# vmoens/mujoco-torch

Hardware: AMD Instinct MI355X
Metric: env-steps/sec (higher is better)
Workload: dtype f64

## Files before the change

### mujoco-torch_amd/csrc/mjh_device.h

```cpp
#pragma once
#include <hip/hip_runtime.h>
#include <stdint.h>

#include "../../include/mjhip.h"

#define MJH_WAVE 64
#define MJH_MAX_DEPTH 128
#define MJH_CHAIN_PRE 3

#define mjMINVAL 1e-15
#define mjMAXVAL 1e10
#define mjMINIMP 1e-4
#define mjMAXIMP 0.9999
#define MINVAL_CACHED ((float)1e-15)

enum { JNT_FREE = 0, JNT_BALL = 1, JNT_SLIDE = 2, JNT_HINGE = 3 };
enum { DSBL_CONSTRAINT = 1 << 0, DSBL_SPRING = 1 << 5, DSBL_DAMPER = 1 << 6, DSBL_GRAVITY = 1 << 7,
       DSBL_CLAMPCTRL = 1 << 8, DSBL_WARMSTART = 1 << 9, DSBL_ACTUATION = 1 << 11, DSBL_REFSAFE = 1 << 12,
       DSBL_EULERDAMP = 1 << 15 };
enum { INT_EULER = 0, INT_RK4 = 1, SOL_CG = 1, SOL_NEWTON = 2, CONE_ELLIPTIC = 1 };
enum { CAM_FIXED = 0, CAM_TRACK = 1, CAM_TRACKCOM = 2, CAM_TARGETBODY = 3, CAM_TARGETBODYCOM = 4 };
enum { GAIN_FIXED = 0, GAIN_AFFINE = 1, GAIN_MUSCLE = 2, BIAS_NONE = 0, BIAS_AFFINE = 1, BIAS_MUSCLE = 2 };
enum { DYN_NONE = 0, DYN_INTEGRATOR = 1, DYN_FILTER = 2, DYN_FILTEREXACT = 3, DYN_MUSCLE = 4 };
#define INLINE_CHOL_MAX 16
// ... 111 lines not shown
  const int* dof_act_id;
  const REAL* dof_act_coef;
  const int* dof_frc_lim;
  const REAL* dof_frc_range;
  const int* dof_act_rot;
  const int* act_ent_adr;
  const int* act_ent_dof;
  const REAL* act_ent_coef;
  const int* act_ent_rot;
  const REAL* ten_J0;
  const REAL* ten_JTAJ;
  int has_ten_armature;
  int con_direct;
  int con_general;
  int act_simple;
  int act_has_rot;
  float inv_nv;
  const int* dof_limrow;
  const int* lim_dof;
  int sol_qm_lds;
  int con_rows;
  int nt_all;
  int all_handoff;
  int lds_diet;
  int crow_by_con;
  int sol2_row_cap;
  int pair_cull_on;
  int sol2_incr;
  int sol2_hs;
  const REAL* crow_par;
  const int* crow_info;
  int ncrow;
  const int* con_body;
  const unsigned long long* con_dmask;
  const REAL* pair_cull;
  const int* cvx_pairs;
  int ncvxpair;
};

__device__ __forceinline__ int lane_id() { return (int)(threadIdx.x & (MJH_WAVE - 1)); }

__device__ __forceinline__ void wave_sync() {
  __builtin_amdgcn_fence(__ATOMIC_RELEASE, "workgroup", "local");
  __builtin_amdgcn_wave_barrier();
  __builtin_amdgcn_fence(__ATOMIC_ACQUIRE, "workgroup", "local");
}
// ... 316 lines not shown
```

### mujoco-torch_amd/csrc/mjh_kernels.h

```cpp
#pragma once
#include <cstring>
#include "mjh_device.h"

template <typename REAL>
struct LdsView {
  REAL* base;
  const LdsOff* off;
#define X(n, c, p) __device__ __forceinline__ REAL* n() const { return base + off->n; }
  MJH_LDS_ARRAYS(X, _)
#undef X
};

#ifndef MJH_NO_NT
#define MJH_NT_STORE(v, p) __builtin_nontemporal_store((v), (p))
#else
#define MJH_NT_STORE(v, p) (*(p) = (v))
#endif
template <typename MM>
inline int lds_carve(const MM& m, int phase_bit, LdsOff& o, int* kv_defer_ok = nullptr) {
  int off = 0;
#define X(n, c, p) o.n = off; if ((p) & phase_bit) off += (((c) + 1) & ~1);
  MJH_LDS_ARRAYS(X, m)
#undef X
  if (phase_bit == PH_CON) {
// ... 78 lines not shown
    o.act = off; off += ev(m.na);
    o.act_dot = off; off += ev(m.na);
    o.con_dist = off; off += ev(m.ncand);
    o.i_con_act = off; off += ev(m.ncon);
    o.i_crow_act = off; off += ev(m.ncon);
    const int rows0 = off, nj = ev(nd * m.nv), n3 = ev(3 * m.ngeom), n9 = ev(9 * m.ngeom);
    o.efc_J = o.efc_Jc = rows0;
    if (n3 + n9 > nj) return -1;
    o.geom_xpos = rows0; o.geom_xmat = rows0 + n3;
    off += nj;
    const int ov = off;
    int ca = ov;
    o.subtree_com = ca; ca += ev(3 * m.nbody);
    o.cdof = ca; ca += ev(6 * m.nv);
    o.con_pos = ca; ca += ev(3 * m.ncand);
    o.con_frame = ca; ca += ev(9 * m.ncand);
    int sa = ov;
    o.efc_D = sa; sa += ev(nd);
    o.efc_aref = sa; sa += ev(nd);
    o.r_vs = sa; sa += ev(m.nv);
    o.r_vs2 = sa; sa += ev(m.nv);
    o.r_pg = sa; sa += ev(2 * m.nv);
    o.r_fs = sa; sa += ev(nd + m.nl);
    const int qpos_at = sa;
    o.qpos = sa; sa += ev(m.nq);
    off = ca > sa ? ca : sa;
    int ta = rows0;
#define X(n, c, p) if ((p) & PH_SOL2T) { o.n = ta; ta += (((c) + 1) & ~1); }
    MJH_LDS_ARRAYS(X, m)
#undef X
    if (ta > qpos_at) return -1;
  }
  if (phase_bit == PH_CRB) {
    const int nn = ((m.nv * m.nv + 1) & ~1);
    if (m.nv <= 32) { o.qLD = 0; if (off < nn) off = nn; }
    else { o.qLD = off; off += nn; }
  }
  return off;
}

template <typename REAL>
struct DevData {
#define X(n) REAL* n;
  MJH_DATA_REALS(X)
#undef X
#define X(n) int32_t* n;
// ... 412 lines not shown
  } else {
#pragma unroll
    for (int k = 0; k < NMAX; k++) T.t[k] = (k < n && valid && k <= i) ? A[(i * (i + 1)) / 2 + k] : (REAL)0;
  }
#pragma unroll
  for (int j = 0; j < NMAX; j++) {
    if (j < n) {
      const REAL sj = dof_read<W, NMAX>(T.t[j], j);
      const REAL dj = r_sqrt<REAL>(sj > (REAL)1e-12 ? sj : (REAL)1e-12);
      const REAL lij = (i == j) ? dj : ((i > j && valid) ? T.t[j] / dj : (REAL)0);
      if (i >= j) T.t[j] = lij;
#pragma unroll
      for (int k = j + 1; k < NMAX; k++) {
        const REAL lkj = dof_read<W, NMAX>(lij, k);
        T.t[k] = (i == j) ? lkj : ((i > j) ? T.t[k] - lij * lkj : T.t[k]);
      }
    }
  }
  REAL dg = 1;
#pragma unroll
  for (int k = 0; k < NMAX; k++) dg = (k == i) ? T.t[k] : dg;
  T.inv = valid ? 1 / dg : (REAL)0;
}
template <int W, typename REAL, int NMAX>
__device__ __forceinline__ void chol_pack_big(TriPack<REAL, NMAX>& T, REAL* colbuf, int n) {
  static_assert(NMAX > 16 && NMAX <= 32 && NMAX <= W, "one lane per row");
  const int i = sub_lane<W>();
  const bool valid = i < n;
#pragma unroll
  for (int j = 0; j < NMAX; j++) {
    if (j < n) {
      const REAL sj = sub_read<W>(T.t[j], j) + (REAL)1e-10;
      const REAL dj = r_sqrt<REAL>(sj);
      const REAL lij = (i == j) ? dj : ((i > j && valid) ? T.t[j] / dj : (REAL)0);
      if (i >= j) T.t[j] = lij;
      REAL* col = colbuf + (j & 1) * NMAX;
      if (i < NMAX) col[i] = lij;
      constexpr int CH = 8;
#pragma unroll
      for (int k0 = 0; k0 < NMAX; k0 += CH) {
        if (k0 + CH - 1 > j) {
          REAL c[CH];
#pragma unroll
          for (int t = 0; t < CH; t++) c[t] = (k0 + t > j && k0 + t < NMAX) ? col[k0 + t] : (REAL)0;
#pragma unroll
          for (int t = 0; t < CH; t++) {
            if (k0 + t > j && k0 + t < NMAX) {
              T.t[k0 + t] = (i == j) ? c[t] : ((i > j) ? T.t[k0 + t] - lij * c[t] : T.t[k0 + t]);
              asm volatile("" : "+v"(T.t[k0 + t]));
            }
          }
        }
      }
    }
  }
  REAL dg = 1;
#pragma unroll
  for (int k = 0; k < NMAX; k++) dg = (k == i) ? T.t[k] : dg;
  T.inv = valid ? 1 / dg : (REAL)0;
}

template <int W, typename REAL, int NMAX>
__device__ __forceinline__ void chol_factor_solve_n(const REAL* A, const REAL* b, REAL* x, int n) {
  TriPack<REAL, NMAX> T;
  chol_factor_pack<W, REAL, NMAX>(A, T, n);
  const int i = sub_lane<W>();
  const REAL xi = tri_solve<W, REAL, NMAX>(T, i < n ? b[i] : (REAL)0, n);
  if (i < n) x[i] = xi;
  wave_sync();
}
template <int W, typename REAL, int NLO = 0, int NHI = 16>
__device__ __forceinline__ void chol_factor_solve(const REAL* A, const REAL* b, REAL* x, int n) {
  if (NLO <= 8 && (NHI <= 8 || n <= 8)) { if constexpr (NLO <= 8) chol_factor_solve_n<W, REAL, 8>(A, b, x, n); }
  else if (NLO <= 12 && NHI > 8 && (NHI <= 12 || n <= 12)) { if constexpr (NLO <= 12 && NHI > 8) chol_factor_solve_n<W, REAL, 12>(A, b, x, n); }
  else { if constexpr (NHI > 12) chol_factor_solve_n<W, REAL, 16>(A, b, x, n); }
}

template <int W, bool APACKED, typename REAL, int NMAX>
__device__ __forceinline__ void chol_factor_reg(const REAL* A, REAL* L, int n) {
  const int i = sub_lane<W>();
  REAL row[NMAX];
#pragma unroll
// ... 571 lines not shown
          for (int i = 0; i < 9; i++) xmb[i] = S.xmat()[9 * b + i];
        }
#pragma unroll
        for (int r = 0; r < 3; r++) {
          const REAL a[3] = {xmb[r], xmb[3 + r], xmb[6 + r]};
          REAL c[3];
          cross3(a, off, c);
          for (int k = 0; k < 3; k++) { S.cdof()[6 * (d + r) + k] = a[k]; S.cdof()[6 * (d + r) + 3 + k] = c[k]; }
        }
      } else if (t == JNT_HINGE) {
        REAL c[3];
        cross3(S.xaxis() + 3 * j, off, c);
        for (int k = 0; k < 3; k++) { S.cdof()[6 * d + k] = S.xaxis()[3 * j + k]; S.cdof()[6 * d + 3 + k] = c[k]; }
      } else {
        for (int k = 0; k < 3; k++) { S.cdof()[6 * d + k] = 0; S.cdof()[6 * d + 3 + k] = S.xaxis()[3 * j + k]; }
      }
    }
    wave_sync();
    STAMP(6);
    if (!(DEFER && W > 16 && M.kv_defer)) com_stores();
    STAMP(7);
  }

  template <bool FUSED = false, int MAXN = (W == 16 ? 16 : 32)>
  __device__ __forceinline__ void crb_factor() {
    const int l = lane_here();
    const int nb = M.nbody, nv = M.nv;
    STAMP0();
    if (!FUSED) {
      REAL* const dst[2] = {S.cinert(), S.cdof()};
      const REAL* const src[2] = {out.cinert, out.cdof};
      const int cnt[2] = {10 * nb, 6 * nv};
      multi_load<W, 2, 3>(dst, src, cnt, e);
    }
    wave_sync();
    STAMP(11);
    for (int w = l; w < nb * 10; w += W) {
      const int b = w / 10, k = w - 10 * b;
      REAL acc = 0;
      if (b > 0) {
        const int end = M.body_subtree_end[b];
        for (int d = end - 1; d >= b; d--) acc += S.cinert()[10 * d + k];
      }
      S.crb()[w] = acc;
    }
    wave_sync();
    STAMP(12);
// ... 8 lines not shown
#pragma unroll
      for (int k = 0; k < 6; k++) s += S.crb_cdof()[6 * i + k] * S.cdof()[6 * j + k];
      if (i == j) s = s + M.dof_armature[i];
      S.qMp()[tri_at<true>(i, j, nv)] = s;
    }
    wave_sync();
    if (M.has_ten_armature) {
      for (int w = l; w < (nv * (nv + 1)) / 2; w += W) S.qMp()[w] = S.qMp()[w] + M.ten_JTAJ[w];
      wave_sync();
    }
    if (out.qM) {
      REAL* gM = out.qM + e * nv * nv;
      for (int w = l; w < nv * nv; w += W) {
        int i, j;
        split_index(w, nv, M.inv_nv, i, j);
        const int hi = i > j ? i : j, lo = i > j ? j : i;
        gM[w] = S.qMp()[(hi * (hi + 1)) / 2 + lo];
      }
    }
    STAMP(14);
    putnt(out.crb, S.crb(), 10 * nb);
    wave_sync();
    STAMP(15);
    chol_factor<W, REAL, MAXN, true>(S.qMp(), S.qLD(), nv);
    STAMP(16);
    put(out.qLD, S.qLD(), nv * nv);
    STAMP(17);
  }

  __device__ __forceinline__ static void plane_sphere_(const REAL* n, const REAL* ppos, const REAL* spos, REAL r, REAL& dist, REAL* pos) {
    const REAL d[3] = {spos[0] - ppos[0], spos[1] - ppos[1], spos[2] - ppos[2]};
    dist = dot3(d, n) - r;
#pragma unroll
    for (int i = 0; i < 3; i++) pos[i] = spos[i] - n[i] * (r + (REAL)0.5 * dist);
  }
  __device__ __forceinline__ static void sphere_sphere_(const REAL* p1, REAL r1, const REAL* p2, REAL r2, REAL& dist, REAL* pos, REAL* n) {
#pragma unroll
    for (int i = 0; i < 3; i++) n[i] = p2[i] - p1[i];
    REAL d = normalize_n<REAL, 3>(n);
    if (d == 0) { n[0] = 1; n[1] = 0; n[2] = 0; }
    d = d - (r1 + r2);
#pragma unroll
    for (int i = 0; i < 3; i++) pos[i] = p1[i] + n[i] * (r1 + d * (REAL)0.5);
    dist = d;
  }
  __device__ __forceinline__ static void closest_segment_point(const REAL* a, const REAL* b, const REAL* pt, REAL* o) {
// ... 2035 lines not shown
    wave_sync();
    row_store<W>(fin.qpos, S.tmp_nq(), M.nq, e);
    row_store<W>(fin.qvel, S.tmp_nv(), M.nv, e);
    if (l == 0 && fin.time) fin.time[e] = time0 + dt;
  }

  template <bool DEFER = false, bool KEEPG = false, bool XK = KEEPG>
  __device__ __forceinline__ void run_kin() {
    STAMP0();
    load_qpos(true);
    wave_sync();
    STAMP(1);
    const bool com_first = XK && (__builtin_popcount((unsigned)blockIdx.x & (unsigned)KA.xswap_k) & 1) != 0;
    kinematics<DEFER, KEEPG, XK>(KA.rk_stage <= 0, com_first);
    if (!com_first) com_pos<DEFER>();
  }
  __device__ __forceinline__ void run_crb() { crb_factor<false>(); }
  __device__ __forceinline__ void run_con() {
    STAMP0();
    if (M.ncon > 0) collision<0, false, true>();
    if (KA.stages & 0x78) make_constraint();
    if (M.ncon > 0 && !(FRIC && M.topk) && !consts_done_) contact_const_stores();
  }
  template <int NMAX>
  __device__ __forceinline__ void sol2_prefetch(Sol2Pre<REAL, NMAX>& P) {
    const int l = lane_here();
    const int nq = M.nq, nv = M.nv, na = M.na;
    const bool dof = l < nv;
    P.f = (dof && out.qfrc_smooth) ? out.qfrc_smooth[e * nv + l] : (REAL)0;
    {
      const REAL* gL = out.qLD + e * nv * nv;
#pragma unroll
      for (int k = 0; k < NMAX; k++) P.T.t[k] = (dof && k < nv) ? (k <= l ? gL[l * nv + k] : gL[k * nv + l]) : (REAL)0;
    }
    P.T.inv = 0;
    const REAL* gq = KA.cur.qpos + e * nq;
#pragma unroll
    for (int j = 0; j < 2; j++) P.qp[j] = l + W * j < nq ? gq[l + W * j] : (REAL)0;
    P.ac = 0; P.ad = 0;
    if (l < na) { const REAL* ga = KA.state_from_cur ? KA.cur.act : in.act; P.ac = ga ? ga[e * na + l] : (REAL)0; P.ad = out.act_dot ? out.act_dot[e * na + l] : (REAL)0; }
    P.warm = (dof && KA.warm_src && M.nefc > 0) ? KA.warm_src[e * nv + l] : (REAL)0;
  }
  template <int NMAX>
  __device__ __forceinline__ void make_constraint_cs(Sol2Pre<REAL, NMAX>& pre, Sol2Con<REAL>& C) {
    const int l = lane_here();
#if MJH_CS_PF >= 2
    {
      const REAL* gq = KA.cur.qpos + e * M.nq;
#pragma unroll
      for (int j = 0; j < 2; j++) pre.qp[j] = l + W * j < M.nq ? gq[l + W * j] : (REAL)0;
    }
#endif
    const int nv = M.nv, nefc = M.nefc, nl = M.nl, ncon = M.ncon, rows = M.con_rows;
    const bool elliptic = M.cone == CONE_ELLIPTIC;
    if (!KA.state_from_cur && KA.do_step) for (int i = l; i < nv; i += W) S.qvel()[i] = checked(S.qvel()[i], (REAL)0);
    REAL lpos = 0, linvw = 0;
    int lj = 0;
    C.jl = 0; C.ldof = 0;
    if (l < nl) {
      lj = M.lim_jnt[l];
      C.ldof = M.jnt_dofadr[lj];
    }
    {
      const int qa = l < nl ? M.jnt_qposadr[lj] : 0;
      const int srcl = (int)(lane_id() & ~(W - 1)) + (qa & (W - 1));
      const REAL q0 = __shfl(pre.qp[0], srcl, MJH_WAVE), q1 = __shfl(pre.qp[1], srcl, MJH_WAVE);
// ... 42 lines not shown
      jac_dof_root(cpos, root1, on1, d, jp1, jr1);
      const REAL dp[3] = {jp2[0] - jp1[0], jp2[1] - jp1[1], jp2[2] - jp1[2]};
      const REAL dr[3] = {jr2[0] - jr1[0], jr2[1] - jr1[1], jr2[2] - jr1[2]};
      REAL diff[6];
#pragma unroll
      for (int r = 0; r < 3; r++) {
        diff[r] = fr[3 * r] * dp[0] + fr[3 * r + 1] * dp[1] + fr[3 * r + 2] * dp[2];
        diff[3 + r] = fr[3 * r] * dr[0] + fr[3 * r + 1] * dr[1] + fr[3 * r + 2] * dr[2];
      }
      REAL* const dst = Jc + (a * rows) * nv + d;
      if (dim == 1) {
        dst[0] = diff[0];
      } else if (!elliptic) {
        const int nedge = 2 * (dim - 1);
        for (int ed = 0; ed < nedge; ed++) {
          const REAL f = fric[ed >> 1] * ((ed & 1) ? (REAL)-1 : (REAL)1);
          dst[ed * nv] = diff[0] + diff[1 + (ed >> 1)] * f;
        }
      } else {
        for (int r = 0; r < dim; r++) dst[r * nv] = diff[r];
      }
    }
#if MJH_CS_PF == 2
    sol2_prefetch<NMAX>(pre);
#endif
    wave_sync();
    STAMP(25);
    C.Dl = 0; C.arl = 0;
    for (int r = l; r < nefc; r += W) {
      REAL solref[2], solimp[5];
      REAL pos = 0, pos_norm = 0, invweight = 0, jv = 0;
      int crow = -1;
      if (r < nl) {
        pos = lpos; pos_norm = lpos; invweight = linvw;
        solref[0] = M.jnt_solref[2 * lj]; solref[1] = M.jnt_solref[2 * lj + 1];
#pragma unroll
        for (int i = 0; i < 5; i++) solimp[i] = M.jnt_solimp[5 * lj + i];
        jv = 0 + C.jl * S.qvel()[C.ldof];
      } else {
        const int q = r - nl, ncr = M.ncrow;
        const int info = M.crow_info[q];
        const REAL* P = M.crow_par + q;
        solref[0] = P[0]; solref[1] = P[ncr];
#pragma unroll
        for (int i = 0; i < 5; i++) solimp[i] = P[(2 + i) * ncr];
        invweight = P[7 * ncr];
        const int c = info & 0xffff, sub = (info >> 16) & 0xff;
// ... 34 lines not shown
      const REAL* Jc = S.efc_Jc();
      REAL* gC = gJ + nl * nv;
      for (int c = 0; c < M.ncon; c++) {
        const int at = slot[c];
        for (int sub = 0; sub < rows; sub += 4) {
          REAL v[4];
#pragma unroll
          for (int t = 0; t < 4; t++) v[t] = (at >= 0 && sub + t < rows && dof) ? Jc[(at * rows + sub + t) * nv + l] : (REAL)0;
#pragma unroll
          for (int t = 0; t < 4; t++) if (sub + t < rows && dof) MJH_NT_STORE(v[t], &gC[(c * rows + sub + t) * nv + l]);
        }
      }
    }
    if (out.efc_frictionloss) for (int r = l; r < nefc; r += W) MJH_NT_STORE((REAL)0, &out.efc_frictionloss[e * nefc + r]);
    if (M.ncon > 0) contact_const_stores();
  }
  template <int NMAX, int RPL, bool ONE = false, bool HANDOFF = false>
  __device__ __forceinline__ void run_con_sol2() {
    static_assert(W == 32 && !FRIC && !DIRECT, "plain constraint stage, two environments per wavefront");
    Sol2Pre<REAL, NMAX> pre;
    Sol2Con<REAL> con;
    STAMP0();
    collision<NMAX, HANDOFF>(&pre);
#if MJH_CS_PF == 1
    sol2_prefetch<NMAX>(pre);
#endif
    make_constraint_cs<NMAX>(pre, con);
#if MJH_CS_PF == 3
    if (HANDOFF && ho_on_) {
      __builtin_amdgcn_fence(__ATOMIC_RELEASE, "workgroup");
      __builtin_amdgcn_fence(__ATOMIC_ACQUIRE, "workgroup");
    }
    sol2_prefetch<NMAX>(pre);
#endif
    wave_sync();
    run_sol2<NMAX, RPL, false, true, ONE>(&pre, &con);
  }
  template <bool FLUID, bool FUSED = false, bool DEFER = false>
  __device__ __forceinline__ void run_vel() {
    STAMP0();
    velocity<FLUID, FUSED, DEFER>();
    if (KA.stages & 0x60) actuation<FLUID>();
    velocity_stores<DEFER>();
  }

  __device__ __forceinline__ void run_sol() {
    const int l = lane_here();
    const int nq = M.nq, nv = M.nv, na = M.na;
    STAMP0();
    load_factor_and_accelerate((KA.stages & 0x40) != 0);
    if (!(KA.stages & 0x40)) return;
    STAMP(53);
    if (M.nefc == 0) {
      for (int d = l; d < nv; d += W) S.qacc()[d] = S.qacc_smooth()[d];
      wave_sync();
      put(out.qacc, S.qacc(), nv);
    } else {
      solve();
    }
    integrate_tail();
  }

  template <int NMAX>
  __device__ __forceinline__ void load_damping_rows(TriPack<REAL, NMAX>& Hh) {
    const int l = lane_here();
    const int nv = M.nv;
    const REAL* gM = out.qM + e * nv * nv;
#pragma unroll
    for (int k = 0; k < NMAX; k++) Hh.t[k] = (l < nv && k <= l) ? gM[k * nv + l] : (REAL)0;
  }
  template <int NLO = 0, int NHI = (1 << 30)>
  __device__ __forceinline__ void integrate_tail() {
    const int l = lane_here();
    const int nq = M.nq, nv = M.nv, na = M.na;
    if (!KA.do_step) return;
    rebind();
    const REAL dt = M.timestep;
    const REAL time0 = in.time ? in.time[e] : (REAL)0;
    const int rk = KA.rk_stage;
    if (rk < 0) {
      const REAL* qacc = S.qacc();
      constexpr bool REGSOL = NHI <= 32;
      if (!(M.disableflags & DSBL_EULERDAMP)) {
        if constexpr (REGSOL && NLO > 16) {
          TriPack<REAL, NHI> Hh;
          load_damping_rows<NHI>(Hh);
          const REAL dd = l < nv ? M.timestep * M.dof_damping[l] : (REAL)0;
          const REAL rhs = l < nv ? S.qfrc_smooth()[l] + (M.nefc ? S.qfrc_constraint()[l] : (in.qfrc_constraint ? in.qfrc_constraint[e * nv + l] : (REAL)0)) : (REAL)0;
#pragma unroll
          for (int k = 0; k < NHI; k++) Hh.t[k] = (k == l) ? Hh.t[k] + dd : Hh.t[k];
          chol_pack_big<W, REAL, NHI>(Hh, S.chol_col(), nv);
          const REAL x = tri_solve<W, REAL, NHI>(Hh, rhs, nv);
          if (l < nv) S.s_Mgrad()[l] = x;
          wave_sync();
        } else {
        REAL* const Hp = REGSOL ? S.H2() : S.H();
        for (int w = l; w < (nv * (nv + 1)) / 2; w += W) {
          int i, j;
          tri_unpack(w, i, j);
          const REAL mw = out.qM[e * nv * nv + i * nv + j];
          Hp[w] = (i == j) ? mw + M.timestep * M.dof_damping[i] : mw;
        }
        for (int d = l; d < nv; d += W) S.s_grad()[d] = S.qfrc_smooth()[d] + (M.nefc ? S.qfrc_constraint()[d] : (in.qfrc_constraint ? in.qfrc_constraint[e * nv + d] : (REAL)0));
        wave_sync();
        if (NLO <= 16 && (NHI <= 16 || nv <= 16)) {
          if constexpr (NLO <= 16) chol_factor_solve<W, REAL, NLO, (NHI < 16 ? NHI : 16)>(Hp, S.s_grad(), S.s_Mgrad(), nv);
        } else {
          if constexpr (NHI > 16 && !REGSOL) {
            chol_factor<W, REAL, 16, true>(S.H(), S.HL(), nv);
            chol_inv_diag<W, false>(S.HL(), S.HL_inv(), nv);
            wave_sync();
            chol_solve<W, false>(S.HL(), S.HL_inv(), S.s_grad(), S.s_Mgrad(), nv);
          }
        }
        }
// ... 26 lines not shown
      for (int i = l; i < nv; i += W) S.tmp_nv2()[i] = a * S.qvel()[i];
      wave_sync();
      for (int i = l; i < nq; i += W) S.qpos()[i] = S.tmp_nq()[i];
      wave_sync();
      integrate_pos(S.qpos(), S.tmp_nv2(), dt, S.tmp_nq());
      for (int i = l; i < na; i += W) KA.nxt.act[e * na + i] = S.act()[i] + (a * S.act_dot()[i]) * dt;
      for (int i = l; i < nv; i += W) KA.nxt.qvel[e * nv + i] = S.s_pgrad()[i] + (a * S.qacc()[i]) * dt;
      wave_sync();
      row_store<W>(KA.nxt.qpos, S.tmp_nq(), nq, e);
      return;
    }
    for (int i = l; i < nv; i += W) { S.s_mv()[i] = RW.sum_qacc[e * nv + i]; S.tmp_nv2()[i] = RW.sum_qvel[e * nv + i]; }
    for (int i = l; i < na; i += W) S.act_dot()[i] = RW.sum_actdot[e * na + i];
    for (int i = l; i < nq; i += W) S.qpos()[i] = S.tmp_nq()[i];
    wave_sync();
    advance(S.qpos(), S.s_pgrad(), S.act(), time0, S.act_dot(), S.s_mv(), S.tmp_nv2());
  }

  template <int NMAX>
  __device__ __forceinline__ REAL tri_solve2(const TriPack<REAL, NMAX>& T, REAL bi) const {
    return tri_solve<W, REAL, NMAX>(T, bi, M.nv);
  }

  template <int NMAX, int RPL, bool NEWTON_ONLY = false, bool CS = false, bool ONE = false>
  __device__ __forceinline__ void run_sol2(const Sol2Pre<REAL, NMAX>* pre = nullptr, const Sol2Con<REAL>* con = nullptr) {
    static_assert(W == 32 || W == 16, "two or four environments per wavefront");
    static_assert(!CS || (W == 32 && !NEWTON_ONLY), "the fused constraint + solver kernel runs two environments per wavefront");
    constexpr bool NEWT = NMAX <= 16;
    const int l = lane_here();
    const int nq = M.nq, nv = M.nv, na = M.na, nefc = M.nefc, nl = M.nl, nd = nefc - nl;
    const bool dof = l < nv, lim = l < nl;
    const bool solving = (KA.stages & 0x40) != 0;
    const bool from_in = !KA.state_from_cur;
    const bool newton = NEWTON_ONLY ? NEWT : (NEWT && M.solver == SOL_NEWTON);
    STAMP0();
    if (KA.row_lo >= 0 && !KA.scan_marks) {
      int rows_active = 0;
      if (solving && nefc > 0) {
        const int ncon = M.ncon;
        const bool elliptic = M.cone == CONE_ELLIPTIC;
        for (int base = 0; base < ncon; base += W) {
          const int c = base + l;
          int rows = 0;
          if (c < ncon) {
            const int dim = M.con_dim[c];
            const bool act = (out.contact_dist[e * ncon + c] - (M.topk ? out.contact_includemargin[e * ncon + c] : M.con_includemargin[c])) < 0;
            rows = act ? (dim == 1 ? 1 : (elliptic ? dim : 2 * (dim - 1))) : 0;
// ... 155 lines not shown
            if (r < nda) { Dd[j] = S.efc_D()[r]; ard[j] = S.efc_aref()[r]; }
          }
          STAMP(83);
        } else if (hsp) {
          STAMP(83);
          const REAL* hJ = hsp + 1 + M.ncon + 2 * nd;
          REAL* dJ = S.efc_Jc();
          const int n = nda * nv;
          for (int i0 = 0; i0 < n; i0 += 16 * W) {
            REAL v[16];
#pragma unroll
            for (int t = 0; t < 16; t++) { const int i = i0 + t * W + l; v[t] = i < n ? hJ[i] : (REAL)0; }
#pragma unroll
            for (int t = 0; t < 16; t++) { const int i = i0 + t * W + l; if (i < n) dJ[i] = v[t]; }
          }
        } else {
#pragma unroll
        for (int j = 0; j < RPL; j++) {
          const int r = l + W * j;
          if (r < nda) { const int x = rsrc[r]; Dd[j] = out.efc_D[e * nefc + x]; ard[j] = out.efc_aref[e * nefc + x]; }
        }
        STAMP(83);
        gather_rows<16>(S.efc_Jc(), gJ, rsrc, nda * nv);
        }
      }
    }
    STAMP(70);
    {
      REAL dg = 1;
#pragma unroll
      for (int k = 0; k < NMAX; k++) dg = (k == l) ? T.t[k] : dg;
      T.inv = dof ? 1 / dg : (REAL)0;
    }
    const REAL qs = tri_solve2<NMAX>(T, f);
    if (dof && out.qacc_smooth) out.qacc_smooth[e * nv + l] = qs;
    STAMP(71);
    if (!solving) return;
    REAL qacc = qs, qfrc = 0;
    if (nefc > 0) {
      const REAL* gM = out.qM + e * nv * nv;
      const REAL scale = (REAL)(M.meaninertia * (double)(nv > 1 ? nv : 1));
      const bool fixed = flags & MJH_FLAG_FIXED_ITERATIONS;
      REAL* vs = S.r_vs();
      REAL* vs2 = S.r_vs2();
      REAL* fs = S.r_fs();
      const REAL* Jc = S.efc_Jc();
// ... 495 lines not shown
        if (lim) MJH_NT_STORE(frl, &out.efc_force[e * nefc + l]);
        if constexpr (CS) {
          const int* slot = reinterpret_cast<const int*>(S.i_crow_act());
          const int rows = M.con_rows;
          const float inv_rows = 1.0f / (float)rows;
          for (int r = l; r < nd; r += W) {
            int c, sub;
            split_index(r, rows, inv_rows, c, sub);
            const int at = slot[c];
            MJH_NT_STORE(at >= 0 ? fs[at * rows + sub] : (REAL)0, &out.efc_force[e * nefc + nl + r]);
          }
        } else
        for (int r = l; r < nd; r += W) { const int q = rdst[r]; MJH_NT_STORE(q != 0xffff ? fs[q] : (REAL)0, &out.efc_force[e * nefc + nl + r]); }
      }
      if constexpr (CS) cs_deferred_stores(*con);
    } else {
      if (dof && out.qacc) out.qacc[e * nv + l] = qacc;
    }
    STAMP(79);
    if (!KA.do_step) return;
    wave_sync();
    if (dof) { S.qacc()[l] = qacc; S.qfrc_smooth()[l] = f; S.qfrc_constraint()[l] = qfrc; }
    wave_sync();
    integrate_tail<(NMAX == 8 ? 0 : (NMAX <= 16 ? 9 : 17)), NMAX>();
  }
};

#undef M
#undef in
#undef out
#undef KA
#undef STAMP
#undef STAMP0

#ifndef MJH_CRB32P_WAVES
#define MJH_CRB32P_WAVES 4
#endif
#ifndef MJH_SOL2_T1_WAVES
#define MJH_SOL2_T1_WAVES 4
#endif
#ifndef MJH_SOL2_W16_WAVES
#define MJH_SOL2_W16_WAVES 4
#endif
#ifndef MJH_CON32D_WAVES
#define MJH_CON32D_WAVES 4
#endif
#ifndef MJH_SOL32_WAVES
// ... 117 lines not shown
        wave_sync();
      }
    }
    __builtin_amdgcn_fence(__ATOMIC_RELEASE, "workgroup");
    __builtin_amdgcn_fence(__ATOMIC_ACQUIRE, "workgroup");
    wave_sync();
    if (idx < K.env_count) {
      REAL* lds3 = reinterpret_cast<REAL*>(lds_raw) + sub * K.lds_reals3;
      Env<REAL, 16, false> E(lds3, K.env_begin + idx, K.flags);
      E.S.off = &K.off3;
      E.template run_sol2<NMAX, RPL, NEWTON_ONLY>();
    }
  } else
  {
    const int64_t idx = blk * NSUB + sub;
    if (idx < K.env_count) {
      Env<REAL, W, false> E(lds, K.env_begin + idx, K.flags);
      if constexpr (ALL) {
        const bool swap_cv = (__builtin_popcount((unsigned)blockIdx.x & (((unsigned)K.flags >> 16) & 0xfffu)) & 1) != 0;
        E.template run_kin<false, true>();
        wave_sync();
        REAL h_qv_early = 0;
        if (!swap_cv) {
          E.template crb_factor<true, NMAX>();
          wave_sync();
          E.template run_vel<false, true>();
        } else {
          E.template run_vel<false, true>();
          wave_sync();
          { const int l_ = (int)(threadIdx.x & (W - 1)); h_qv_early = l_ < K.M.nv ? E.S.qvel()[l_] : (REAL)0; }
          wave_sync();
          E.template crb_factor<true, NMAX>();
          wave_sync();
        }
        if (K.M.all_handoff) {
          const int l = (int)(threadIdx.x & (W - 1));
          const int nv6 = 6 * K.M.nv, nb3 = 3 * K.M.nbody, ng = K.M.ngeom;
          REAL h_cd[6], h_sc[3], h_qv;
#pragma unroll
          for (int k = 0; k < 6; k++) h_cd[k] = l + W * k < nv6 ? E.S.cdof()[l + W * k] : (REAL)0;
#pragma unroll
          for (int k = 0; k < 3; k++) h_sc[k] = l + W * k < nb3 ? E.S.subtree_com()[l + W * k] : (REAL)0;
          h_qv = swap_cv ? h_qv_early : (l < K.M.nv ? E.S.qvel()[l] : (REAL)0);
          wave_sync();
          E.S.off = &K.off2;
#pragma unroll
          for (int k = 0; k < 6; k++) if (l + W * k < nv6) E.S.cdof()[l + W * k] = h_cd[k];
#pragma unroll
          for (int k = 0; k < 3; k++) if (l + W * k < nb3) E.S.subtree_com()[l + W * k] = h_sc[k];
          if (l < K.M.nv) E.S.qvel()[l] = h_qv;
          if (l < ng) {
#pragma unroll
            for (int i = 0; i < 3; i++) E.S.geom_xpos()[3 * l + i] = E.ho_g[i];
#pragma unroll
            for (int i = 0; i < 9; i++) E.S.geom_xmat()[9 * l + i] = E.ho_g[3 + i];
// ... 46 lines not shown
```

### mujoco-torch_amd/csrc/mjhip.hip

```cpp
#include <hip/hip_runtime.h>

#include <algorithm>
#include <cstdio>
#include <cstdlib>
#include <cstring>
#include <string>
#include <vector>

#include "mjh_kernels.h"
#include "mjh_convex.h"
#include "mjh_sensor.h"
#include "mjh_reset.h"
#include "mjh_io.h"
#include "mjh_inverse.h"
#include "mjh_ray.h"
#include "mjh_render.h"
#include "mjh_support.h"
#include "mjh_fd.h"
#include "mjh_instances.h"

#define X_(R, P, W) extern template __global__ void mjh_phase_kernel<R, P, W>(KArgs<R>);
#define S_(R, N, RPL, W) extern template __global__ void mjh_sol2_kernel<R, N, RPL, W>(KArgs<R>);
#define C_(R) extern template __global__ void mjh_convex_kernel<R>(KArgs<R>);
#define N_(R) extern template __global__ void mjh_sensor_kernel<R, 0>(KArgs<R>); extern template __global__ void mjh_sensor_kernel<R, 1>(KArgs<R>);
// ... 181 lines not shown
const char* const kStageLeaves[] = {
    "qpos", "qvel", "act", "qacc_warmstart", "qacc", "act_dot", "xipos", "geom_xpos", "geom_xmat", "subtree_com", "cdof",
    "cinert", "qM", "qLD", "efc_J", "efc_D", "efc_aref", "qfrc_smooth", "qacc_smooth", "qfrc_constraint",
    "contact_dist" };
const char* const kConvexStageLeaves[] = {"contact_dist", "contact_pos", "contact_frame"};
const char* const kEqStageLeaves[] = {"xpos", "xquat", "xmat"};
bool is_stage_leaf(const char* name, bool has_convex, bool has_fluid, bool has_eq, bool topk) {
  if (topk && !strcmp(name, "contact_includemargin")) return true;
  if (!strcmp(name, "qfrc_gravcomp") || !strncmp(name, "ten_", 4)) return false;
  if (has_eq) for (const char* s : kEqStageLeaves) if (!strcmp(s, name)) return true;
  for (const char* s : kStageLeaves) if (!strcmp(s, name)) return true;
  if (has_convex) for (const char* s : kConvexStageLeaves) if (!strcmp(s, name)) return true;
  if (has_fluid && !strcmp(name, "ximat")) return true;
  return false;
}

bool on(const char* e) { return !(e && e[0] == '0'); }
int tri(const char* e) { return !e ? -1 : (e[0] == '1' ? 1 : 0); }
int mask12(const char* e) { return e ? (int)(strtol(e, nullptr, 0) & 0xfff) : -1; }
int num(const char* e, int unset) { return e ? atoi(e) : unset; }
struct Switches {
  bool all_handoff = on(getenv("MJH_ALL_HANDOFF"));
  bool lds_diet = on(getenv("MJH_LDS_DIET"));
  bool pair_cull = on(getenv("MJH_PAIR_CULL"));
  bool kin_level = on(getenv("MJH_KIN_LEVEL"));
  bool sol2_mfma = on(getenv("MJH_SOL2_MFMA"));
  bool sol2_incr = on(getenv("MJH_SOL2_INCR"));
  bool handover = on(getenv("MJH_HANDOVER"));
  int kcv2 = tri(getenv("MJH_KCV2"));
  int fuse_all = tri(getenv("MJH_FUSE_ALL"));
  bool fuse_stage = on(getenv("MJH_FUSE_STAGE"));
  bool fuse_stage0 = on(getenv("MJH_FUSE_STAGE0"));
  bool fuse_tail = on(getenv("MJH_FUSE_TAIL"));
  bool cs_one = on(getenv("MJH_CS_ONE"));
  int xswap = mask12(getenv("MJH_XSWAP"));
  int xswap_k = mask12(getenv("MJH_XSWAP_K"));
  int xswap_c = mask12(getenv("MJH_XSWAP_C"));
  int sensor_epw = num(getenv("MJH_SENSOR_EPW"), 0);
  int max_grid_log2 = std::min(std::max(num(getenv("MJH_MAX_GRID_LOG2"), 20), 0), 20);
};
const Switches& switches() {
  static const Switches s;
  return s;
}

constexpr int kLdsCu = 160 * 1024;
// ... 327 lines not shown
    else if (fn == MJH_FN_CAPSULE_CONVEX) need = 6 * d->convex_nfv[c2];
    else if (fn == MJH_FN_CONVEX_CONVEX) {
      const int K = d->convex_nfv[c1] > d->convex_nfv[c2] ? d->convex_nfv[c1] : d->convex_nfv[c2];
      need = 3 * (d->convex_nvert[c1] + d->convex_nface[c1] + d->convex_nvert[c2] + d->convex_nface[c2]) + 43 * K;
    }
    if (need > cvx_reals) cvx_reals = need;
    cvx_pairs.push_back(p);
  }
  fix.push_back({(const void**)&M.cvx_pairs, bb.add(cvx_pairs.data(), sizeof(int) * cvx_pairs.size())});
  M.ncvxpair = (int)cvx_pairs.size();
  out->cvx_lds_bytes = (cvx_reals + 8) * (int)sizeof(REAL);
  if (out->cvx_lds_bytes > kLdsWg) return fail(-12, "convex hull too large for the pair kernel's LDS scratch");
  for (int i = 0; i < nv; i++) if (d->dof_damping[i] != 0) out->any_damping = 1;
  out->leaf_count = leaf_counts(d);
  return 0;
}

template <typename REAL>
int plan(const mjhModelDesc* d, mjhModel* out, DevModel<REAL>& M) {
  const Switches& sw = switches();
  const int nv = d->nv;
  M.con_direct = (nv <= 16 && !M.con_general) ? 1 : 0;
  M.all_handoff = (sw.all_handoff && d->ngeom <= 32 && d->nbody <= 32 && nv <= 32) ? 1 : 0;
  M.lds_diet = (sw.lds_diet && d->nbody <= 16 && d->njnt <= 16 && nv <= 16 && !M.has_fluid && !M.has_gravcomp && d->ntendon == 0) ? 1 : 0;
  M.pair_cull_on = sw.pair_cull ? 1 : 0;
  M.kin_lvl = (sw.kin_level && d->nbody > 1 && d->nbody <= 32) ? 1 : 0;
  M.sol_qm_lds = (d->nefc > 0 && d->iterations > 4) ? 1 : 0;
  M.sol2_hs = (sw.sol2_mfma && sizeof(REAL) == 4 && d->solver == SOL_NEWTON && nv <= 16 && d->nefc > 0) ? 1 : 0;
  M.sol2_incr = (sw.sol2_incr && d->solver == SOL_NEWTON && nv <= 16 && d->nefc > 0) ? 1 : 0;

  for (int p = 0; p < MJH_NARENA; p++) {
    carve(out, (Arena)p, M, 1 << p);
    if (p == AR_SOL && out->lds(AR_SOL) > kLdsCu && M.sol_qm_lds) {
      M.sol_qm_lds = 0;
      carve(out, AR_SOL, M, 1 << p);
    }
    if (p < MJH_NPHASE && out->lds((Arena)p) > kLdsCu) return fail(-12, "model does not fit the 160 KiB LDS of one CU");
  }
  {
    const int nd = d->nefc - d->nf - d->nl;
    const bool general = d->nf > 0 || d->nft > 0 || d->ne > 0 || d->nlb > 0 || d->nlt > 0;
    const int nmax = nv <= 8 ? 8 : (nv <= 16 ? 16 : 28), rpl = nd <= 32 ? 1 : (nd <= 64 ? 2 : (nd <= 128 ? 4 : 8));
    const bool w16 = nv <= 16 && d->na <= 16 && d->nl <= 16;
    const bool solver_ok = d->solver == SOL_CG || (d->solver == SOL_NEWTON && (nv <= 8 || w16));
    if (solver_ok && !general && nv <= 28 && nd <= 32 * (nmax <= 16 ? 8 : 2) && d->nl <= 32 && d->na <= 32 && d->nq <= 64 && 2 * out->lds(AR_SOL2) <= kLdsWg) {
      out->sol2_nmax = nmax;
// ... 948 lines not shown
  }
  if (kernel == MJH_KERNEL_FD_PERTURB || kernel == MJH_KERNEL_FD_DIFFERENCE) {
    const int64_t R = f64 ? 8 : 4, nq = f64 ? m->m64.nq : m->m32.nq, nv = f64 ? m->m64.nv : m->m32.nv, na = f64 ? m->m64.na : m->m32.na, nu = f64 ? m->m64.nu : m->m32.nu;
    const int64_t nb = f64 ? m->m64.nbody : m->m32.nbody, nmo = f64 ? m->m64.nmocap : m->m32.nmocap, nsd = f64 ? m->m64.nsensordata : m->m32.nsensordata, neq = f64 ? m->m64.neq : m->m32.neq;
    if (kernel == MJH_KERNEL_FD_PERTURB) {
      read_write_bytes[0] = read_write_bytes[1] = (1 + nq + 5 * nv + na + 2 * nu + 6 * nb + 7 * nmo + 3 * nb + nsd + 18 * nb) * R + 4 * neq;
    } else {
      read_write_bytes[0] = (nq + nv + na + nsd) * R;
      read_write_bytes[1] = (2 * nv + na + nsd) * R;
    }
    return 0;
  }
  if (kernel == MJH_KERNEL_INVERSE) {
    const int64_t R = f64 ? 8 : 4, nv = f64 ? m->m64.nv : m->m32.nv, nefc = f64 ? m->m64.nefc : m->m32.nefc;
    read_write_bytes[0] = (nefc * nv + 2 * nefc + nv * nv + 3 * nv) * R;
    read_write_bytes[1] = (nefc + 2 * nv) * R;
    return 0;
  }
  if (kernel == MJH_KERNEL_PASS) {
    if (!m->fuse_all) return -2;
    int64_t a13[2] = {0, 0}, a14[2] = {0, 0};
    if (kernel_io(m, MJH_KERNEL_KCV, a13, true, stages13) != 0 || kernel_io(m, MJH_KERNEL_CS, a14, true, stages13) != 0) return -2;
    read_write_bytes[0] = a13[0] + a14[0]; read_write_bytes[1] = a13[1] + a14[1];
    return 0;
  }
  if (kernel == MJH_KERNEL_STAGE) {
    if (!m->fuse_stage) return -2;
    int64_t a13[2] = {0, 0}, a8[2] = {0, 0}, a9[2] = {0, 0};
    if (kernel_io(m, MJH_KERNEL_KCV, a13, true, true) != 0 || kernel_io(m, MJH_KERNEL_CON_DIRECT, a8, true, true) != 0 || kernel_io(m, MJH_KERNEL_SOL2, a9, true, true) != 0) return -2;
    read_write_bytes[0] = a13[0] + a8[0] + a9[0]; read_write_bytes[1] = a13[1] + a8[1] + a9[1];
    return 0;
  }
  if (kernel == MJH_KERNEL_TAIL) {
    if (!m->fuse_tail) return -2;
    int64_t a8[2] = {0, 0}, a9[2] = {0, 0};
    if (kernel_io(m, MJH_KERNEL_CON_DIRECT, a8, true, stages13) != 0 || kernel_io(m, MJH_KERNEL_SOL2, a9, true, stages13) != 0) return -2;
    read_write_bytes[0] = a8[0] + a9[0]; read_write_bytes[1] = a8[1] + a9[1];
    return 0;
  }
  if ((kernel == MJH_KERNEL_KCV || kernel == MJH_KERNEL_CS) && m->fuse_all && !inner) return -2;
  if (kernel == MJH_KERNEL_CS) {
    if (!m->fuse_cs) return -2;
    int64_t k2[2] = {0, 0}, k4[2] = {0, 0};
    if (io_of(MJH_KERNEL_CON, k2) != 0 || io_of(MJH_KERNEL_SOL, k4) != 0) return -2;
    const int64_t R = f64 ? 8 : 4, nv = f64 ? m->m64.nv : m->m32.nv, nefc = f64 ? m->m64.nefc : m->m32.nefc, nl = f64 ? m->m64.nl : m->m32.nl;
    read_write_bytes[0] = k2[0] + k4[0] - ((nefc - nl) * nv + 2 * nefc + nl + nv) * R;
// ... 67 lines not shown
```

Baseline: 30.46 million.

## Pair mass-matrix and damped Cholesky factorizations inside the whole-pass solver

Adds an opt-in mode for 17-28 DOF models in which crb_factor skips its Cholesky. The solver prefetches qM directly and factors both M and M+h*damping in one interleaved pass, writing qLD back from registers. The Euler tail then reuses the damped factor instead of reloading and refactoring it. f64 square roots in this path use a hardware rsq seed plus Newton steps. It adds register pressure and an LDS scratch reservation, and the interleaving may change accuracy slightly.

After: 29.28 million. 3.9% lower.

```diff
diff --git a/mujoco-torch_amd/csrc/mjh_device.h b/mujoco-torch_amd/csrc/mjh_device.h
--- a/mujoco-torch_amd/csrc/mjh_device.h
+++ b/mujoco-torch_amd/csrc/mjh_device.h
@@ -157,6 +157,7 @@
   int con_rows;
   int nt_all;
   int all_handoff;
+  int pair_factor;
   int lds_diet;
   int crow_by_con;
   int sol2_row_cap;
diff --git a/mujoco-torch_amd/csrc/mjh_kernels.h b/mujoco-torch_amd/csrc/mjh_kernels.h
--- a/mujoco-torch_amd/csrc/mjh_kernels.h
+++ b/mujoco-torch_amd/csrc/mjh_kernels.h
@@ -124,6 +124,7 @@
     o.r_vs2 = sa; sa += ev(m.nv);
     o.r_pg = sa; sa += ev(2 * m.nv);
     o.r_fs = sa; sa += ev(nd + m.nl);
+    if (m.pair_factor && sa < o.r_vs + 4 * 28) sa = o.r_vs + 4 * 28;
     const int qpos_at = sa;
     o.qpos = sa; sa += ev(m.nq);
     off = ca > sa ? ca : sa;
@@ -582,7 +583,21 @@
   for (int k = 0; k < NMAX; k++) dg = (k == i) ? T.t[k] : dg;
   T.inv = valid ? 1 / dg : (REAL)0;
 }
-template <int W, typename REAL, int NMAX>
+template <bool RSQ, typename REAL>
+__device__ __forceinline__ REAL chol_big_scale(REAL sj, REAL tj, bool diag, bool below) {
+  if constexpr (RSQ && sizeof(REAL) == 8) {
+    const double sd = (double)sj, hs = 0.5 * sd;
+    double y = __builtin_amdgcn_rsq(sd);
+    y = y * (1.5 - hs * y * y);
+    y = y * (1.5 - hs * y * y);
+    const REAL d = (REAL)(sd * y);
+    return diag ? d : (below ? tj * (REAL)y : (REAL)0);
+  } else {
+    const REAL dj = r_sqrt<REAL>(sj);
+    return diag ? dj : (below ? tj / dj : (REAL)0);
+  }
+}
+template <int W, typename REAL, int NMAX, bool RSQ = false>
 __device__ __forceinline__ void chol_pack_big(TriPack<REAL, NMAX>& T, REAL* colbuf, int n) {
   static_assert(NMAX > 16 && NMAX <= 32 && NMAX <= W, "one lane per row");
   const int i = sub_lane<W>();
@@ -591,8 +606,7 @@
   for (int j = 0; j < NMAX; j++) {
     if (j < n) {
       const REAL sj = sub_read<W>(T.t[j], j) + (REAL)1e-10;
-      const REAL dj = r_sqrt<REAL>(sj);
-      const REAL lij = (i == j) ? dj : ((i > j && valid) ? T.t[j] / dj : (REAL)0);
+      const REAL lij = chol_big_scale<RSQ, REAL>(sj, T.t[j], i == j, i > j && valid);
       if (i >= j) T.t[j] = lij;
       REAL* col = colbuf + (j & 1) * NMAX;
       if (i < NMAX) col[i] = lij;
@@ -618,6 +632,56 @@
 #pragma unroll
   for (int k = 0; k < NMAX; k++) dg = (k == i) ? T.t[k] : dg;
   T.inv = valid ? 1 / dg : (REAL)0;
+}
+template <int W, typename REAL, int NMAX, bool RSQ_A, int J>
+__device__ __forceinline__ void chol_pack_big2_step(TriPack<REAL, NMAX>& Ta, TriPack<REAL, NMAX>& Tb, REAL* colbuf_a, REAL* colbuf_b, int n, int i, bool valid) {
+  if constexpr (J < NMAX) {
+    constexpr int j = J;
+    if (j < n) {
+      const REAL sa = sub_read<W>(Ta.t[j], j) + (REAL)1e-10;
+      const REAL sb = sub_read<W>(Tb.t[j], j) + (REAL)1e-10;
+      const REAL la = chol_big_scale<RSQ_A, REAL>(sa, Ta.t[j], i == j, i > j && valid);
+      const REAL lb = chol_big_scale<false, REAL>(sb, Tb.t[j], i == j, i > j && valid);
+      if (i >= j) { Ta.t[j] = la; Tb.t[j] = lb; }
+      REAL* cola = colbuf_a + (j & 1) * NMAX;
+      REAL* colb = colbuf_b + (j & 1) * NMAX;
+      if (i < NMAX) { cola[i] = la; colb[i] = lb; }
+      constexpr int CH = 8;
+#pragma unroll
+      for (int k0 = 0; k0 < NMAX; k0 += CH) {
+        if (k0 + CH - 1 > j) {
+          REAL ca[CH], cb[CH];
+#pragma unroll
+          for (int t = 0; t < CH; t++) {
+            ca[t] = (k0 + t > j && k0 + t < NMAX) ? cola[k0 + t] : (REAL)0;
+            cb[t] = (k0 + t > j && k0 + t < NMAX) ? colb[k0 + t] : (REAL)0;
+          }
+#pragma unroll
+          for (int t = 0; t < CH; t++) {
+            if (k0 + t > j && k0 + t < NMAX) {
+              Ta.t[k0 + t] = (i == j) ? ca[t] : ((i > j) ? Ta.t[k0 + t] - la * ca[t] : Ta.t[k0 + t]);
+              Tb.t[k0 + t] = (i == j) ? cb[t] : ((i > j) ? Tb.t[k0 + t] - lb * cb[t] : Tb.t[k0 + t]);
+              asm volatile("" : "+v"(Ta.t[k0 + t]));
+              asm volatile("" : "+v"(Tb.t[k0 + t]));
+            }
+          }
+        }
+      }
+    }
+    chol_pack_big2_step<W, REAL, NMAX, RSQ_A, J + 1>(Ta, Tb, colbuf_a, colbuf_b, n, i, valid);
+  }
+}
+template <int W, typename REAL, int NMAX, bool RSQ_A>
+__device__ __forceinline__ void chol_pack_big2(TriPack<REAL, NMAX>& Ta, TriPack<REAL, NMAX>& Tb, REAL* colbuf_a, REAL* colbuf_b, int n) {
+  static_assert(NMAX > 16 && NMAX <= 32 && NMAX <= W, "one lane per row");
+  const int i = sub_lane<W>();
+  const bool valid = i < n;
+  chol_pack_big2_step<W, REAL, NMAX, RSQ_A, 0>(Ta, Tb, colbuf_a, colbuf_b, n, i, valid);
+  REAL da = 1, db = 1;
+#pragma unroll
+  for (int k = 0; k < NMAX; k++) { da = (k == i) ? Ta.t[k] : da; db = (k == i) ? Tb.t[k] : db; }
+  Ta.inv = valid ? 1 / da : (REAL)0;
+  Tb.inv = valid ? 1 / db : (REAL)0;
 }
 
 template <int W, typename REAL, int NMAX>
@@ -1235,7 +1299,7 @@
     STAMP(7);
   }
 
-  template <bool FUSED = false, int MAXN = (W == 16 ? 16 : 32)>
+  template <bool FUSED = false, int MAXN = (W == 16 ? 16 : 32), bool PAIRK = false>
   __device__ __forceinline__ void crb_factor() {
     const int l = lane_here();
     const int nb = M.nbody, nv = M.nv;
@@ -1290,6 +1354,7 @@
     putnt(out.crb, S.crb(), 10 * nb);
     wave_sync();
     STAMP(15);
+    if (PAIRK && M.pair_factor) { STAMP(16); STAMP(17); return; }
     chol_factor<W, REAL, MAXN, true>(S.qMp(), S.qLD(), nv);
     STAMP(16);
     put(out.qLD, S.qLD(), nv * nv);
@@ -3371,13 +3436,17 @@
     if (KA.stages & 0x78) make_constraint();
     if (M.ncon > 0 && !(FRIC && M.topk) && !consts_done_) contact_const_stores();
   }
-  template <int NMAX>
+  template <int NMAX, bool PAIRK = false>
   __device__ __forceinline__ void sol2_prefetch(Sol2Pre<REAL, NMAX>& P) {
     const int l = lane_here();
     const int nq = M.nq, nv = M.nv, na = M.na;
     const bool dof = l < nv;
     P.f = (dof && out.qfrc_smooth) ? out.qfrc_smooth[e * nv + l] : (REAL)0;
-    {
+    if (PAIRK && M.pair_factor) {
+      const REAL* gM = out.qM + e * nv * nv;
+#pragma unroll
+      for (int k = 0; k < NMAX; k++) P.T.t[k] = (dof && k <= l) ? gM[k * nv + l] : (REAL)0;
+    } else {
       const REAL* gL = out.qLD + e * nv * nv;
 #pragma unroll
       for (int k = 0; k < NMAX; k++) P.T.t[k] = (dof && k < nv) ? (k <= l ? gL[l * nv + k] : gL[k * nv + l]) : (REAL)0;
@@ -3390,7 +3459,7 @@
     if (l < na) { const REAL* ga = KA.state_from_cur ? KA.cur.act : in.act; P.ac = ga ? ga[e * na + l] : (REAL)0; P.ad = out.act_dot ? out.act_dot[e * na + l] : (REAL)0; }
     P.warm = (dof && KA.warm_src && M.nefc > 0) ? KA.warm_src[e * nv + l] : (REAL)0;
   }
-  template <int NMAX>
+  template <int NMAX, bool PAIRK = false>
   __device__ __forceinline__ void make_constraint_cs(Sol2Pre<REAL, NMAX>& pre, Sol2Con<REAL>& C) {
     const int l = lane_here();
 #if MJH_CS_PF >= 2
@@ -3479,7 +3548,7 @@
       }
     }
 #if MJH_CS_PF == 2
-    sol2_prefetch<NMAX>(pre);
+    sol2_prefetch<NMAX, PAIRK>(pre);
 #endif
     wave_sync();
     STAMP(25);
@@ -3560,19 +3629,21 @@
     Sol2Con<REAL> con;
     STAMP0();
     collision<NMAX, HANDOFF>(&pre);
+    constexpr bool PAIRK = HANDOFF && NMAX > 16 && ONE;
+    static_assert(!PAIRK || MJH_CS_PF != 0, "the narrow phase's own prefetch does not know the instantiation");
 #if MJH_CS_PF == 1
-    sol2_prefetch<NMAX>(pre);
+    sol2_prefetch<NMAX, PAIRK>(pre);
 #endif
-    make_constraint_cs<NMAX>(pre, con);
+    make_constraint_cs<NMAX, PAIRK>(pre, con);
 #if MJH_CS_PF == 3
     if (HANDOFF && ho_on_) {
       __builtin_amdgcn_fence(__ATOMIC_RELEASE, "workgroup");
       __builtin_amdgcn_fence(__ATOMIC_ACQUIRE, "workgroup");
     }
-    sol2_prefetch<NMAX>(pre);
+    sol2_prefetch<NMAX, PAIRK>(pre);
 #endif
     wave_sync();
-    run_sol2<NMAX, RPL, false, true, ONE>(&pre, &con);
+    run_sol2<NMAX, RPL, false, true, ONE, PAIRK>(&pre, &con);
   }
   template <bool FLUID, bool FUSED = false, bool DEFER = false>
   __device__ __forceinline__ void run_vel() {
@@ -3607,8 +3678,8 @@
 #pragma unroll
     for (int k = 0; k < NMAX; k++) Hh.t[k] = (l < nv && k <= l) ? gM[k * nv + l] : (REAL)0;
   }
-  template <int NLO = 0, int NHI = (1 << 30)>
-  __device__ __forceinline__ void integrate_tail() {
+  template <int NLO = 0, int NHI = (1 << 30), bool PAIRK = false>
+  __device__ __forceinline__ void integrate_tail(const TriPack<REAL, (PAIRK ? NHI : 1)>* Hd = nullptr, bool paired = false) {
     const int l = lane_here();
     const int nq = M.nq, nv = M.nv, na = M.na;
     if (!KA.do_step) return;
@@ -3621,14 +3692,19 @@
       constexpr bool REGSOL = NHI <= 32;
       if (!(M.disableflags & DSBL_EULERDAMP)) {
         if constexpr (REGSOL && NLO > 16) {
-          TriPack<REAL, NHI> Hh;
-          load_damping_rows<NHI>(Hh);
-          const REAL dd = l < nv ? M.timestep * M.dof_damping[l] : (REAL)0;
           const REAL rhs = l < nv ? S.qfrc_smooth()[l] + (M.nefc ? S.qfrc_constraint()[l] : (in.qfrc_constraint ? in.qfrc_constraint[e * nv + l] : (REAL)0)) : (REAL)0;
-#pragma unroll
-          for (int k = 0; k < NHI; k++) Hh.t[k] = (k == l) ? Hh.t[k] + dd : Hh.t[k];
-          chol_pack_big<W, REAL, NHI>(Hh, S.chol_col(), nv);
-          const REAL x = tri_solve<W, REAL, NHI>(Hh, rhs, nv);
+          REAL x = 0;
+          bool have = false;
+          if constexpr (PAIRK) if (paired) { x = tri_solve<W, REAL, NHI>(*Hd, rhs, nv); have = true; }
+          if (!have) {
+            TriPack<REAL, NHI> Hh;
+            load_damping_rows<NHI>(Hh);
+            const REAL dd = l < nv ? M.timestep * M.dof_damping[l] : (REAL)0;
+#pragma unroll
+            for (int k = 0; k < NHI; k++) Hh.t[k] = (k == l) ? Hh.t[k] + dd : Hh.t[k];
+            chol_pack_big<W, REAL, NHI>(Hh, S.chol_col(), nv);
+            x = tri_solve<W, REAL, NHI>(Hh, rhs, nv);
+          }
           if (l < nv) S.s_Mgrad()[l] = x;
           wave_sync();
         } else {
@@ -3701,7 +3777,7 @@
     return tri_solve<W, REAL, NMAX>(T, bi, M.nv);
   }
 
-  template <int NMAX, int RPL, bool NEWTON_ONLY = false, bool CS = false, bool ONE = false>
+  template <int NMAX, int RPL, bool NEWTON_ONLY = false, bool CS = false, bool ONE = false, bool PAIRK = false>
   __device__ __forceinline__ void run_sol2(const Sol2Pre<REAL, NMAX>* pre = nullptr, const Sol2Con<REAL>* con = nullptr) {
     static_assert(W == 32 || W == 16, "two or four environments per wavefront");
     static_assert(!CS || (W == 32 && !NEWTON_ONLY), "the fused constraint + solver kernel runs two environments per wavefront");
@@ -3903,6 +3979,28 @@
         }
         STAMP(83);
         gather_rows<16>(S.efc_Jc(), gJ, rsrc, nda * nv);
+        }
+      }
+    }
+    TriPack<REAL, (PAIRK ? NMAX : 1)> Hd;
+    bool paired = false;
+    if constexpr (PAIRK) {
+      static_assert(CS && NMAX <= 28, "the whole-pass kernel's solver");
+      if (M.pair_factor) {
+        paired = KA.do_step && KA.rk_stage < 0 && !(M.disableflags & DSBL_EULERDAMP);
+        REAL* const cb = S.r_vs();
+        if (paired) {
+          const REAL dd = l < nv ? M.timestep * M.dof_damping[l] : (REAL)0;
+#pragma unroll
+          for (int k = 0; k < NMAX; k++) Hd.t[k] = (k == l) ? T.t[k] + dd : T.t[k];
+          chol_pack_big2<W, REAL, NMAX, true>(T, Hd, cb, cb + 2 * NMAX, nv);
+        } else {
+          chol_pack_big<W, REAL, NMAX, true>(T, cb, nv);
+        }
+        if (out.qLD) {
+          REAL* gL = out.qLD + e * nv * nv;
+#pragma unroll
+          for (int r = 0; r < NMAX; r++) if (dof && r < nv) gL[r * nv + l] = (l <= r) ? T.t[r] : (REAL)0;
         }
       }
     }
@@ -4444,7 +4542,7 @@
     wave_sync();
     if (dof) { S.qacc()[l] = qacc; S.qfrc_smooth()[l] = f; S.qfrc_constraint()[l] = qfrc; }
     wave_sync();
-    integrate_tail<(NMAX == 8 ? 0 : (NMAX <= 16 ? 9 : 17)), NMAX>();
+    integrate_tail<(NMAX == 8 ? 0 : (NMAX <= 16 ? 9 : 17)), NMAX, PAIRK>(&Hd, paired);
   }
 };
 
@@ -4608,7 +4706,7 @@
         wave_sync();
         REAL h_qv_early = 0;
         if (!swap_cv) {
-          E.template crb_factor<true, NMAX>();
+          E.template crb_factor<true, NMAX, (NMAX > 16 && ONE)>();
           wave_sync();
           E.template run_vel<false, true>();
         } else {
@@ -4616,7 +4714,7 @@
           wave_sync();
           { const int l_ = (int)(threadIdx.x & (W - 1)); h_qv_early = l_ < K.M.nv ? E.S.qvel()[l_] : (REAL)0; }
           wave_sync();
-          E.template crb_factor<true, NMAX>();
+          E.template crb_factor<true, NMAX, (NMAX > 16 && ONE)>();
           wave_sync();
         }
         if (K.M.all_handoff) {
diff --git a/mujoco-torch_amd/csrc/mjhip.hip b/mujoco-torch_amd/csrc/mjhip.hip
--- a/mujoco-torch_amd/csrc/mjhip.hip
+++ b/mujoco-torch_amd/csrc/mjhip.hip
@@ -227,6 +227,7 @@
 struct Switches {
   bool all_handoff = on(getenv("MJH_ALL_HANDOFF"));
   bool lds_diet = on(getenv("MJH_LDS_DIET"));
+  int pair_factor = tri(getenv("MJH_PAIR_FACTOR"));
   bool pair_cull = on(getenv("MJH_PAIR_CULL"));
   bool kin_level = on(getenv("MJH_KIN_LEVEL"));
   bool sol2_mfma = on(getenv("MJH_SOL2_MFMA"));
@@ -600,6 +601,7 @@
   const int nv = d->nv;
   M.con_direct = (nv <= 16 && !M.con_general) ? 1 : 0;
   M.all_handoff = (sw.all_handoff && d->ngeom <= 32 && d->nbody <= 32 && nv <= 32) ? 1 : 0;
+  M.pair_factor = (sw.pair_factor == 1 && nv > 16 && nv <= 28) ? 1 : 0;
   M.lds_diet = (sw.lds_diet && d->nbody <= 16 && d->njnt <= 16 && nv <= 16 && !M.has_fluid && !M.has_gravcomp && d->ntendon == 0) ? 1 : 0;
   M.pair_cull_on = sw.pair_cull ? 1 : 0;
   M.kin_lvl = (sw.kin_level && d->nbody > 1 && d->nbody <= 32) ? 1 : 0;
@@ -1594,6 +1596,11 @@
     int64_t a13[2] = {0, 0}, a14[2] = {0, 0};
     if (kernel_io(m, MJH_KERNEL_KCV, a13, true, stages13) != 0 || kernel_io(m, MJH_KERNEL_CS, a14, true, stages13) != 0) return -2;
     read_write_bytes[0] = a13[0] + a14[0]; read_write_bytes[1] = a13[1] + a14[1];
+    {
+      const int64_t R = f64 ? 8 : 4, nv = f64 ? m->m64.nv : m->m32.nv;
+      const int pair = (f64 ? m->m64.pair_factor : m->m32.pair_factor) && (f64 ? m->m64.iterations : m->m32.iterations) == 1, dis = f64 ? m->m64.disableflags : m->m32.disableflags;
+      if (pair && !rk4 && !(dis & DSBL_EULERDAMP)) read_write_bytes[0] -= nv * (nv + 1) / 2 * R;
+    }
     return 0;
   }
   if (kernel == MJH_KERNEL_STAGE) {
```
